# drwangxian/viterbi_spl

Hardware: AMD Instinct MI355X
Metric: Viterbi Mframes/s at S=361 T=30k; achieved HBM GB/s vs peak (higher is better)
Workload: dtype f32

## Files before the change

viterbi_spl_amd/csrc/banded.hip:

```cpp
#include "device_common.hpp"

namespace vit {

template <int W, int NWT, bool DW, bool DBG, int NXT, typename ET>
__global__ void __launch_bounds__((NWT + (DW ? 3 : 2)) * 64) banded_forward_kernel(FwdArgs a) {
    extern __shared__ __align__(16) unsigned char smem[];
    constexpr int NP = NWT * 64;
    constexpr int EPL = NWT;
    const int S = a.S, SP = a.SP, T = a.T, SD = a.SD;
    constexpr int DC = NP + 16;
    float* dls = reinterpret_cast<float*>(smem);
    float* dl = dls + 4;
    float* Pv = dls + 4 * DC;
    float* Sv = Pv + NP + 1;
    float* Dv = Sv + NP + 1;
    VI* tot = reinterpret_cast<VI*>(Dv + kMaxDenseRows);

    const int tid = threadIdx.x;
    const int lane = tid & 63;
    const int wv = __builtin_amdgcn_readfirstlane(tid >> 6);
    const int song = blockIdx.x;
    const int Tb = song_length(a.lengths, song, T);
    const ET* __restrict__ E = reinterpret_cast<const ET*>(a.logE) + (size_t)song * T * S;
    float* __restrict__ hist = a.hist + (size_t)song * T * SD;
// ... 182 lines not shown
        }
        const unsigned long long s3 = prof ? stamp() : 0ull;
        __syncthreads();
        if (prof) {
            const unsigned long long s4 = stamp();
            ph0 += s1 - s0; ph1 += s2 - s1; ph2 += s3 - s2; ph3 += s4 - s3;
        }
    };
    const unsigned long long clk0 = (dbg & 48) ? __builtin_amdgcn_s_memtime() : 0ull;
    const unsigned long long rt0 = (dbg & 48) ? __builtin_amdgcn_s_memrealtime() : 0ull;
    int t = 1;
    for (; t + 1 < Tb; t += 2) {
        frame(t, e_a);
        frame(t + 1, e_b);
    }
    if (t < Tb) frame(t, e_a);

    terminal_argmax(is_target ? dl[j] : -INFINITY, j, tvalid, tot, NWT + (DW ? 3 : 2), a.last_state, a.loglik, song);
    if ((dbg & 256) && lane == 0 && Tb > 1) {
        float* o = a.fmax + (size_t)song * 64 + 4 * wv;
        const float n = (float)(Tb - 1);
        o[0] = (float)ph0 / n; o[1] = (float)ph1 / n; o[2] = (float)ph2 / n; o[3] = (float)ph3 / n;
    }
    if ((dbg & 48) && tid == 0) {
        const unsigned long long d = (dbg & 16) ? __builtin_amdgcn_s_memtime() - clk0 : __builtin_amdgcn_s_memrealtime() - rt0;
        a.fmax[(size_t)song * 64 + 63] = (float)d / (float)(Tb > 1 ? Tb - 1 : 1);
    }
}

#include "banded_floor.inc"

constexpr int split_waitcnt(int vm, int lgkm) { return (vm & 15) | ((vm >> 4) << 14) | (7 << 4) | (lgkm << 8); }
constexpr int kNoVmWait = 63;
template <int... K, typename F>
__device__ __forceinline__ void split_frames(std::integer_sequence<int, K...>, F&& f) { (f(std::integral_constant<int, K>{}), ...); }
template <int NXT, int PF, typename ET, bool WPR = false, bool XQ = false>
__global__ void __launch_bounds__(64 * (kSplitFullWaves + kSplitHalfWaves)) banded_floor_split_forward_kernel(FwdArgs a) {
    extern __shared__ __align__(16) unsigned char smem[];
    constexpr int W = 32;
    constexpr int NWF = kSplitFullWaves, NW = kSplitFullWaves + kSplitHalfWaves;
    using L = FloorSplitLds;
    constexpr int DC = L::DC, BUF = L::BUF;
    float* dls = reinterpret_cast<float*>(smem) + L::dls;
    float* fmg = dls + L::fmg;
    VI* tot = reinterpret_cast<VI*>(dls + L::tot);
    const int S = a.S, SP = a.SP, T = a.T, SD = a.SD;
    constexpr bool GEN = NXT < 0;
    constexpr int NXL = GEN ? kMaxExtras : NXT;
    const int nx = GEN ? a.n_extras : NXT;

    const int tid = threadIdx.x;
    const int lane = tid & 63;
    const int wv = __builtin_amdgcn_readfirstlane(tid >> 6);
    const bool half = wv >= NWF;
    const int hh = half ? lane >> 5 : 0;
    const int song = blockIdx.x;
    const int Tb = song_length(a.lengths, song, T);
    const ET* __restrict__ E = reinterpret_cast<const ET*>(a.logE) + (size_t)song * T * S;
    float* __restrict__ hist = a.hist + (size_t)song * T * SD;

    const int j = half ? 64 * NWF + 32 * (wv - NWF) + (lane & 31) : tid;
    const bool tvalid = j < S;
    const bool own = tvalid && hh == 0;
    const int jc = tvalid ? j : 0;
    const int jld = tvalid ? j : S - 1;
    const bool is_fm = j == S;
    const unsigned hoff = tvalid ? (unsigned)(SD + j) : (is_fm ? (unsigned)S : (unsigned)(SD + S + 1));
    const unsigned hoffb = 4u * hoff, eoffb = (unsigned)(sizeof(ET) * jld);
    const int lo = reinterpret_cast<const int32_t*>(a.image + a.off_lo)[jc];
    int xcol[NXL > 0 ? NXL : 1];
    bool is_x = false;
#pragma unroll
    for (int k = 0; k < NXL; ++k) {
        xcol[k] = k < nx ? a.extras[k] : 0;
        is_x |= (k < nx && j == xcol[k]);
    }
    const int sh = a.win_shift;
    const int lov = (tvalid ? lo : 0) + sh;
    const float* rp = dls + 4 + (lov & 3) * DC + (lov & ~3) + 16 * hh;
    float* fmp = fmg + fm_slot((XQ && is_x) ? (lane | 1) : lane);
    static_assert(!XQ || NXT == 1, "the extra column leaves M by address only where the launcher proved its quad idle");

    for (int k = tid; k < L::reset; k += NW * 64) dls[k] = -INFINITY;
    __syncthreads();

#ifdef VIT_TIMING_HOOKS
    const bool probe = (a.debug & 48) != 0;
    constexpr bool wprobe = WPR;
    WaveProbe wp_;
#else
    constexpr bool probe = false;
#endif
    unsigned long long clk0 = 0ull, rt0 = 0ull;

    auto body = [&](auto role, auto resets) {
        constexpr bool HALF = decltype(role)::value, RESETS = decltype(resets)::value;
        constexpr int WL = HALF ? W / 2 : W;
        const float cj = own ? reinterpret_cast<const float*>(a.image + a.off_rowc)[jc] : -INFINITY;
        float aw[WL];
        float xa[NXL > 0 ? NXL : 1];
        {
            const float* __restrict__ tab = reinterpret_cast<const float*>(a.image + a.off_tabA);
            const float* __restrict__ xaT = reinterpret_cast<const float*>(a.image + a.off_extraA);
#pragma unroll
            for (int w = 0; w < WL; ++w) aw[w] = tvalid ? tab[(size_t)(w + (HALF ? 16 * hh : 0)) * SP + jc] : -INFINITY;
#pragma unroll
            for (int k = 0; k < NXL; ++k)
                xa[k] = (tvalid && k < nx && (!HALF || hh == 1)) ? xaT[(size_t)k * SP + jc] : -INFINITY;
        }
        float* wp = dls + 4 + sh + j + (HALF ? hh * split_upper_off(DC) : 0);
        int xo[NXL > 0 ? NXL : 1];
#pragma unroll
        for (int k = 0; k < NXL; ++k) {
            xo[k] = 4 + sh + xcol[k];
            asm volatile("" : "+v"(xo[k]));
        }

        auto produce = [&](const float dn, const int WB, const int G, const int Z) {
#pragma unroll
            for (int c = 0; c < (HALF ? 2 : 4); ++c) wp[WB * BUF + floor_copy_off(DC, c)] = dn;
            fm_publish(fmp + G * kFmGroupFloats, (!XQ && NXL > 0 && is_x) ? -INFINITY : dn);
            if constexpr (RESETS) fmg[Z * kFmGroupFloats + lane] = -INFINITY;
        };

        {
            const float d0 = tvalid ? reinterpret_cast<const float*>(a.image + a.off_logpi)[j] + load_e<ET>(E + j) : -INFINITY;
            if (own) hist[j] = d0;
            produce(d0, 0, 0, 1);
        }
        float er[PF];
#pragma unroll
        for (int k = 0; k < PF; ++k) er[k] = load_e<ET>(E + (size_t)(1 + k < Tb ? 1 + k : Tb - 1) * S + jld);
#pragma unroll
        for (int w = 0; w < WL; ++w) asm volatile("" ::"v"(aw[w]));
#pragma unroll
        for (int k = 0; k < NXL; ++k) asm volatile("" ::"v"(xa[k]));
        asm volatile("" ::"v"(cj));
        __syncthreads();

        const unsigned rowH = 4u * (unsigned)SD, rowE = (unsigned)sizeof(ET) * (unsigned)S;
        float* hb = hist;
        const ET* eb = E;
        unsigned elim = 0;
        auto round_bases = [&](const int t) {
            const int r = t + PF < Tb ? t + PF : Tb - 1;
            const int ahead = Tb - 1 - r < PF ? Tb - 1 - r : PF;
            hb = hist + (size_t)(t - 1) * SD;
            eb = E + (size_t)r * S;
            elim = (unsigned)ahead * rowE;
        };
        auto frame = [&](float& e_slot, auto uc) {
            constexpr int u = decltype(uc)::value;
            const int RB = u & 1, WB = RB ^ 1;
            const int GR = u % kFmGroups, GW = (u + 1) % kFmGroups, GZ = (u + 2) % kFmGroups;
            const f32x4* __restrict__ win = reinterpret_cast<const f32x4*>(rp + RB * BUF);
            float xd[NXL > 0 ? NXL : 1];
            f32x4 fq;
            float m0, m1 = -INFINITY, m2 = -INFINITY, m3 = -INFINITY;
#pragma unroll
            for (int k = 0; k < NXL; ++k) xd[k] = dls[xo[k] + RB * BUF];
            fq = reinterpret_cast<const f32x4*>(fmg + GR * kFmGroupFloats)[0];
            asm volatile("" ::: "memory");
            f32x4 dw[WL / 4];
#pragma unroll
            for (int q = 0; q < WL / 4; ++q) dw[q] = win[q];
            __builtin_amdgcn_sched_barrier(0);
            const float M = fmaxf(fmaxf(fq.x, fq.y), fmaxf(fq.z, fq.w));
            m0 = M + cj;
            asm volatile("" ::"v"(m0));
            __builtin_amdgcn_sched_barrier(0);
            split_frames(std::make_integer_sequence<int, WL / 8>{}, [&](auto gc) {
                constexpr int w = 8 * decltype(gc)::value;
                constexpr bool last = w + 8 == WL;
                constexpr int vmw = PF - 1 + u;
                static_assert(vmw <= 2 * (PF - 1) && 2 * (PF - 1) < kNoVmWait, "vmcnt bound: one store and one load per frame, 6-bit field");
                constexpr bool pairw = w + 16 >= WL && w >= 8;
                f32x4 da = dw[w / 4], db = dw[w / 4 + 1];
                if constexpr (pairw) {
                    __builtin_amdgcn_s_waitcnt(split_waitcnt(last ? vmw : kNoVmWait, last ? 0 : 2));
                    asm volatile("" : "+v"(da), "+v"(db));
                }
                f32x2 c0_ = f32x2{da.x, da.y} + f32x2{aw[w + 0], aw[w + 1]};
                f32x2 c1_ = f32x2{da.z, da.w} + f32x2{aw[w + 2], aw[w + 3]};
                f32x2 c2_ = f32x2{db.x, db.y} + f32x2{aw[w + 4], aw[w + 5]};
                f32x2 c3_ = f32x2{db.z, db.w} + f32x2{aw[w + 6], aw[w + 7]};
                asm volatile("" : "+v"(c0_), "+v"(c1_), "+v"(c2_), "+v"(c3_));
                m0 = fmaxf(fmaxf(m0, c0_.x), c0_.y);
                m1 = fmaxf(fmaxf(m1, c1_.x), c1_.y);
                m2 = fmaxf(fmaxf(m2, c2_.x), c2_.y);
                m3 = fmaxf(fmaxf(m3, c3_.x), c3_.y);
            });
#pragma unroll
            for (int k = 0; k < NXL; ++k) m1 = fmaxf(m1, xd[k] + xa[k]);
            float mx = fmaxf(fmaxf(m0, m1), fmaxf(m2, m3));
            if constexpr (HALF) mx = max_other_half(mx);
            const float dn = mx + e_slot;
#ifdef VIT_TIMING_HOOKS
            if constexpr (wprobe) wp_.before_publish(dn);
#endif
            const float sv = (HALF && is_fm) ? M : dn;
            const unsigned eso = (unsigned)u * rowE < elim ? (unsigned)u * rowE : elim;
            produce(dn, WB, GW, GZ);
            asm volatile("" ::: "memory");
            row_store_f32(hb, hoffb, sv, (unsigned)u * rowH);
            e_slot = row_load_e<ET>(eb, eoffb, eso);
#ifdef VIT_TIMING_HOOKS
            if constexpr (wprobe) wp_.barrier(); else
#endif
            __syncthreads();
        };
#ifdef VIT_TIMING_HOOKS
        if constexpr (wprobe) wp_.start();
#endif
        clk0 = probe ? __builtin_amdgcn_s_memtime() : 0ull;
        rt0 = probe ? __builtin_amdgcn_s_memrealtime() : 0ull;
        if constexpr (HALF) __builtin_amdgcn_s_setprio(1);
        int t = 1;
        for (; t + PF - 1 < Tb; t += PF) {
            round_bases(t);
            split_frames(std::make_integer_sequence<int, PF>{}, [&](auto k) { frame(er[k], k); });
        }
        round_bases(t);
        split_frames(std::make_integer_sequence<int, PF - 1>{}, [&](auto k) {
            if (t + k < Tb) frame(er[k], k);
        });
    };
    static_assert(PF % 2 == 0 && PF % kFmGroups == 0, "the unrolled frames must cycle through whole buffer and slot-group rounds");
// ... 194 lines not shown
        __syncthreads();
        if (tid == 0) {
            VI acc = vi_identity();
            for (int b = 0; b < NPW; ++b) acc = op_fwd(acc, tot[b]);
            if (acc.i == kBig) acc.i = 0;
            a.last_state[song] = acc.i;
            if (a.loglik) a.loglik[song] = acc.v;
        }
    }
    if (probe && tid == 0) {
        const unsigned long long d = (a.debug & 16) ? __builtin_amdgcn_s_memtime() - clk0 : __builtin_amdgcn_s_memrealtime() - rt0;
        a.fmax[(size_t)song * 64 + 63] = (float)d / (float)(Tb > 1 ? Tb - 1 : 1);
    }
}

__global__ void scan_selftest_kernel(const float* __restrict__ vals, int mode, float* __restrict__ out_v,
                                     int32_t* __restrict__ out_i) {
    const int j = threadIdx.x + blockIdx.x * blockDim.x;
    VI x{vals[j], (int)threadIdx.x};
    if (mode == 0) x = wave_scan<false>(x);
    else if (mode == 1) x = wave_scan<true>(x);
    else if (mode == 2) x.v = wave_scan_max(x.v);
    else if (mode == 3) x.v = wave_shift_up(wave_scan_max(x.v), -INFINITY);
    else x.v = wave_max_all(x.v);
    out_v[j] = x.v;
    out_i[j] = x.i;
}

template <int W, int NWT, typename ET>
static hipError_t launch_floor_t(const FwdArgs& a, hipStream_t st) {
    constexpr int PF = floor_pf<W>();
    if constexpr (W == 32 && NWT == 6) {
        static_assert(kSplitStates == NWT * 64, "the split kernel keeps the six-wave kernel's LDS and history layout");
        if (a.fwd_form == 6 || (a.fwd_form == 0 && a.B <= 256 && std::is_same_v<ET, float>)) {
            constexpr size_t ldss = FloorSplitLds::bytes();
            constexpr int NWS = kSplitFullWaves + kSplitHalfWaves;
            const bool xq = a.n_extras == 1 && a.extras[0] == a.S - 1 && (a.S - 1) % 4 == 0;
#ifdef VIT_TIMING_HOOKS
            if ((a.debug & 64) && xq)
                hipLaunchKernelGGL((banded_floor_split_forward_kernel<1, PF, ET, true, true>), dim3((int)a.B), dim3(NWS * 64), ldss, st, a);
            else if ((a.debug & 64) && a.n_extras == 1)
                hipLaunchKernelGGL((banded_floor_split_forward_kernel<1, PF, ET, true>), dim3((int)a.B), dim3(NWS * 64), ldss, st, a);
            else
#endif
            if (xq)
                hipLaunchKernelGGL((banded_floor_split_forward_kernel<1, PF, ET, false, true>), dim3((int)a.B), dim3(NWS * 64), ldss, st, a);
            else if (a.n_extras == 1)
                hipLaunchKernelGGL((banded_floor_split_forward_kernel<1, PF, ET>), dim3((int)a.B), dim3(NWS * 64), ldss, st, a);
            else
                hipLaunchKernelGGL((banded_floor_split_forward_kernel<-1, PF, ET>), dim3((int)a.B), dim3(NWS * 64), ldss, st, a);
            return hipGetLastError();
        }
    }
    if constexpr (W <= 32 && NWT <= 8) {
        const bool pair = a.pair_ok && ((a.B > 256 && a.fwd_form != 1 && a.fwd_form != 6) || a.fwd_form == 2);
        if (pair) {
            constexpr int NPW = (NWT + 1) / 2;
            constexpr int PFP = 4;
            constexpr size_t ldsp = FloorPairLds<NPW>::bytes();
            if (W == 32 && a.n_extras == 1)
                hipLaunchKernelGGL((banded_floor_pair_forward_kernel<W, NPW, (W == 32 ? 1 : -1), PFP, ET>), dim3((int)a.B), dim3(NPW * 64), ldsp, st, a);
            else
                hipLaunchKernelGGL((banded_floor_pair_forward_kernel<W, NPW, -1, PFP, ET>), dim3((int)a.B), dim3(NPW * 64), ldsp, st, a);
            return hipGetLastError();
        }
    }
    constexpr size_t ldsf = FloorLds<W, NWT>::bytes();
#ifdef VIT_TIMING_HOOKS
    if constexpr (W == 32 && NWT == 6) {
        if ((a.debug & 64) && a.n_extras == 1) {
            hipLaunchKernelGGL((banded_floor_forward_kernel<W, NWT, 1, PF, ET, WgVariant::Plain, true>), dim3((int)a.B), dim3(NWT * 64), ldsf, st, a);
            return hipGetLastError();
        }
    }
#endif
    return with_nxt<W>(a.n_extras, [&](auto nxt) {
        hipLaunchKernelGGL((banded_floor_forward_kernel<W, NWT, decltype(nxt)::value, PF, ET>), dim3((int)a.B), dim3(NWT * 64), ldsf, st, a);
        return hipGetLastError();
    });
}

// ... 63 lines not shown
```

viterbi_spl_amd/csrc/capi.hip:

```cpp
#include <hip/hip_runtime.h>

#include <algorithm>
#include <cstdlib>
#include <cstring>
#include <functional>
#include <mutex>
#include <queue>
#include <new>
#include <utility>
#include <vector>

#include "../../include/viterbi_hip.h"
#include "kernels.hpp"
#include "plan.hpp"

struct Tuning {
    int forward_form = 0;
    int backtrace_form = 0;
    int dense_songs = 0;
    int dense_one_thread = 0;
    int dense_form = 0;
    int step_form = 0;
    int bt_chunks = 0;
    int bt_warm = -1;
    int win_shift = -1;
    int wave_min_batch = 0;
    int wave_two = 0;
    int wave_uniform = 0;
    int bt_fast_rows = 0;
    int bt_block_waves = 0;
    int wave_history = 0;
    int timing = 0;
};

enum Family : int {
    kFamNone = 0,
    kFamStep = 1,
    kFamGroup = 2,
    kFamWave = 3,
};
inline hipError_t launch_family(int family, vit::WgVariant v, const vit::FwdArgs& a, bool f16, hipStream_t st) {
    if (family == kFamWave) return vit::launch_wave(a, f16, st);
    return family == kFamGroup ? vit::launch_banded_variant(a, v, f16, st) : vit::launch_step_variant(a, v, f16, st);
}

struct HistLayout {
    int SD = 0;
    int col0 = 0, mcol = 0;
    int xcol0 = -1;
    int have_fmax = 0;
};

struct FwdStamp {
    const void* ws = nullptr;
    int64_t B = 0, T = 0;
    int family = 0;
    HistLayout lay;
    int aux_frames = 1;
    int half = 0;
    const void* logE = nullptr;
    int e_f16 = 0;
};

// ... 209 lines not shown
    info->reserved[2] = (plan->bp.ok && plan->bp.lo_affine ? 1 : 0) | (plan->bp.ok && plan->bp.pair_ok ? 2 : 0) |
                        (plan->bp.step_ok && vit::step_kernel_instantiated(plan->S, plan->bp.step_bw, plan->bp.step_kb) ? 4 : 0) |
                        (plan->bp.ok && plan->bp.wave_ok ? 8 : 0);
    info->consts[0] = plan->bp.c0;
    for (int k = 0; k < vit::kMaxExtras; ++k) info->extras[k] = k < plan->bp.n_extras ? plan->bp.extras[k] : -1;
    return VIT_OK;
}

size_t vit_plan_image_bytes(const vit_plan* plan) { return plan ? plan->L.bytes : 0; }

int vit_plan_upload(vit_plan* plan, void* device_image, size_t bytes, vit_stream stream) {
    if (!plan || !device_image) return VIT_EINVAL;
    if (bytes < plan->L.bytes || ((uintptr_t)device_image & 255) != 0) return VIT_EINVAL;
    VIT_TRY(hipMemcpyAsync(device_image, plan->host_image.data(), plan->L.bytes, hipMemcpyHostToDevice, (hipStream_t)stream));
    plan->dev_image = static_cast<const uint8_t*>(device_image);
    int dev = 0, cus = 0;
    if (hipGetDevice(&dev) == hipSuccess && hipDeviceGetAttribute(&cus, hipDeviceAttributeMultiprocessorCount, dev) == hipSuccess && cus > 0)
        plan->n_cus = cus;
    return VIT_OK;
}

size_t vit_workspace_bytes(const vit_plan* plan, int64_t B, int64_t T) {
    if (!plan || B < 0 || T < 1) return 0;
    return ws_layout(plan, B, T).bytes;
}

static int* tuning_field(Tuning& t, const char* key) {
    struct { const char* k; int Tuning::*f; } const tab[] = {
        {"forward_form", &Tuning::forward_form}, {"backtrace_form", &Tuning::backtrace_form},
        {"dense_songs", &Tuning::dense_songs}, {"dense_one_thread", &Tuning::dense_one_thread}, {"dense_form", &Tuning::dense_form},
        {"step_form", &Tuning::step_form}, {"bt_chunks", &Tuning::bt_chunks}, {"bt_warm", &Tuning::bt_warm},
        {"win_shift", &Tuning::win_shift}, {"wave_min_batch", &Tuning::wave_min_batch}, {"wave_two", &Tuning::wave_two},
        {"bt_fast_rows", &Tuning::bt_fast_rows}, {"bt_block_waves", &Tuning::bt_block_waves}, {"wave_history", &Tuning::wave_history}, {"wave_uniform", &Tuning::wave_uniform},
        {"timing", &Tuning::timing},
    };
    for (const auto& e : tab)
        if (std::strcmp(e.k, key) == 0) return &(t.*(e.f));
    return nullptr;
}

int vit_plan_set_option(vit_plan* plan, const char* key, int64_t value) {
    if (!plan || !key) return VIT_EINVAL;
    if (std::strcmp(key, "reset") == 0) { plan->tune = Tuning(); return VIT_OK; }
    int* f = tuning_field(plan->tune, key);
    if (!f || value < -1 || value > (int64_t)1 << 30) return VIT_EINVAL;
#ifndef VIT_TIMING_HOOKS
    if (f == &plan->tune.timing && value != 0) return VIT_EUNSUPPORTED;
#endif
    *f = (int)value;
    return VIT_OK;
}

static int resolve_family(const vit_plan* plan, int algo, int64_t B) {
    const int nwt = vit::banded_waves_for(plan->S);
    const bool group_ok = plan->bp.ok && (vit::scan_form_instantiated(plan->bp.W, nwt) ||
                                          (plan->bp.floor_ok && plan->S < nwt * 64 && vit::floor_form_instantiated(plan->bp.W, nwt)));
    const bool wave_ok = plan->bp.ok && plan->bp.wave_ok;
    const int ff = plan->tune.forward_form;
    const int64_t wmin = plan->tune.wave_min_batch > 0 ? plan->tune.wave_min_batch : wave_min_batch(plan);
    if (algo == VIT_ALGO_DENSE) return kFamStep;
    if (algo == VIT_ALGO_WAVE) return wave_ok ? kFamWave : VIT_EUNSUPPORTED;
    if (algo == VIT_ALGO_GROUP) return group_ok ? kFamGroup : VIT_EUNSUPPORTED;
    if (algo != VIT_ALGO_AUTO && algo != VIT_ALGO_BANDED) return VIT_EINVAL;
    const bool want_wave = wave_ok && ff != 5 && (ff == 4 || (ff == 0 && B >= wmin) || !group_ok);
    if (want_wave) return kFamWave;
    if (group_ok) return kFamGroup;
    return algo == VIT_ALGO_AUTO ? kFamStep : VIT_EUNSUPPORTED;
// ... 13 lines not shown
    a.c0 = plan->bp.c0;
    a.debug = tn.timing;
    a.fwd_form = (tn.forward_form >= 1 && tn.forward_form <= 3) || tn.forward_form == 6 ? tn.forward_form : 0;
    a.dense_kt1 = tn.dense_one_thread;
    a.dense_form = tn.dense_form;
    a.step_form = tn.step_form;
    a.off_logpi = plan->L.off_logpi;
    a.off_A4 = plan->L.off_A4;
    a.off_lo = plan->L.off_lo;
    a.off_kind = plan->L.off_kind;
    a.off_tabA = plan->L.off_tabA;
    a.off_extraA = plan->L.off_extraA;
    a.off_denseA = plan->L.off_denseA;
    a.off_rowc = plan->L.off_rowc;
    a.off_lo2 = plan->L.off_lo2;
    a.off_tabP = plan->L.off_tabP;
    a.pair_ok = plan->bp.ok && plan->bp.pair_ok ? 1 : 0;
    a.floor_ok = plan->bp.ok && plan->bp.floor_ok ? 1 : 0;
    a.step_ok = plan->bp.step_ok ? 1 : 0;
    a.step_bw = plan->bp.step_bw;
    a.step_kb = plan->bp.step_kb;
    a.step_cn = plan->bp.step_cn;
    a.off_stepC = plan->L.off_stepC;
    a.off_Arow = plan->L.off_Arow;
    a.off_tabV = plan->L.off_tabV;
    a.wave_ok = plan->bp.ok && plan->bp.wave_ok ? 1 : 0;
    a.wave_npl = plan->bp.wave_npl;
    a.wave_dk = plan->bp.wave_dk;
    a.wave_u5 = tn.wave_uniform == 1 ? 0 : (tn.wave_uniform == 2 ? (plan->wave_u5 >= 1 ? 1 : 0) : (tn.wave_uniform == 3 && plan->wave_u5 == 2 ? 3 : plan->wave_u5));
    a.wave_flags = ((tn.wave_two & 3) == 1 ? 1 : ((tn.wave_two & 3) == 2 ? 2 : 0)) | (tn.wave_two & 4);
    a.win_shift = (plan->bp.ok && plan->bp.lo_affine) ? (plan->bp.lo_off & 3) : 0;
    a.win_shift2 = (plan->bp.ok && plan->bp.pair_ok && plan->bp.lo2_affine) ? (plan->bp.lo2_off & 3) : 0;
    if (tn.win_shift >= 0) a.win_shift = a.win_shift2 = tn.win_shift & 3;
}

size_t vit_workspace_bytes_for(const vit_plan* plan, int64_t B, int64_t T, int algo) {
    if (!plan || B < 0 || T < 1) return 0;
    const int family = resolve_family(plan, algo, B);
    if (family < 0) return 0;
    return ws_layout_family(plan, family, B, T).bytes;
}

int vit_forward(const vit_plan* plan, const void* logE, int emis_dtype, int64_t B, int64_t T,
                const int64_t* lengths, void* workspace, size_t workspace_bytes, float* loglik, int algo,
                vit_stream stream) {
    int rc = check_common(plan, B, T, workspace);
    if (rc != VIT_OK) return rc;
    if (!logE) return VIT_EINVAL;
    if (emis_dtype != VIT_F32 && emis_dtype != VIT_F16) return VIT_EINVAL;
    const int family = resolve_family(plan, algo, B);
    if (family < 0) return family;
    const Tuning& tn = plan->tune;
    const bool half = family == kFamWave && wave_half_applies(plan, T);
    if (family == kFamWave && tn.wave_history == 2 && !half && T >= 2) return VIT_EUNSUPPORTED;
    const WsLayout w = ws_layout_family(plan, family, B, T);
    if (workspace_bytes < w.bytes) return VIT_EWORKSPACE;
    if (B == 0) return VIT_OK;
    stamp_erase(plan, workspace);

    uint8_t* ws = static_cast<uint8_t*>(workspace);
    vit::FwdArgs a{};
    fwd_args_from_plan(plan, a);
    a.logE = logE;
    a.lengths = lengths;
    a.hist = reinterpret_cast<float*>(ws + w.off_hist);
    a.fmax = reinterpret_cast<float*>(ws + w.off_fmax);
// ... 900 lines not shown
```

viterbi_spl_amd/csrc/kernels.hpp:

```cpp
#pragma once
#include <hip/hip_runtime.h>

#include <cstdint>

#include "plan.hpp"

namespace vit {

constexpr int banded_waves_for(int S) {
    const int need = (S + 63) / 64;
    const int opts[5] = {2, 4, 6, 8, 12};
    for (int k = 0; k < 5; ++k)
        if (opts[k] >= need) return opts[k];
    return 0;
}
constexpr bool scan_form_instantiated(int W, int nwt) { return nwt > 0 && ((W <= 32 && nwt <= 12) || (W == 64 && nwt <= 6)); }
constexpr bool floor_form_instantiated(int W, int nwt) { return nwt > 0 && W <= 128 && nwt <= 12; }
constexpr int banded_target_waves(int S, int W) {
    const int nwt = banded_waves_for(S);
    return scan_form_instantiated(W, nwt) ? nwt : 0;
}
enum class WgVariant { Plain, Packed, Ckpt, PackedCkpt };
constexpr bool floor_packed_applies(int S, int W, bool floor_ok, int n_dense) {
    const int nwt = banded_waves_for(S);
// ... 19 lines not shown
    int T, S, SP, S4, SD, W;
    int n_extras, n_dense;
    int extras[kMaxExtras];
    float c0;
    int debug;
    int fwd_form;
    int dense_kt1;
    int dense_form;
    int step_form;
    size_t off_logpi, off_A4, off_lo, off_kind, off_tabA, off_extraA, off_denseA, off_rowc, off_lo2, off_tabP;
    int pair_ok;
    int floor_ok;
    int step_ok, step_bw, step_kb;
    float step_cn;
    size_t off_stepC, off_Arow;
    int win_shift2;
    size_t off_tabV;
    int wave_ok, wave_npl, wave_dk;
    int wave_u5;
    int wave_flags;
    int hist_half;
    int64_t hist_rows;
    int ckpt_every, t_begin, t_end;
    const float* init_rows;
    int64_t init_stride;
    const int64_t* offsets;
    int n_slots;
    const int32_t* slot_begin;
    const int32_t* slot_songs;
    const int64_t* ckpt_base;
    const int32_t* unit_song;
    const int32_t* unit_seg;
    int win_shift;
};

struct BtArgs {
    const uint8_t* image;
    const float* hist;
    const int32_t* last_state;
    const int64_t* lengths;
    int32_t* states;
    int32_t* entry;
    int64_t B;
    int T, S, SP, SD, W, K;
    int col0, mcol;
    int xcol0;
    int aux_frames;
    int chunks, warm;
    int banded;
    int have_fmax;
    int bt_form;
    int lo_affine, lo_off;
    int dense_rows[kMaxDenseRows];
    int n_extras, n_dense;
    int extras[kMaxExtras];
    float c0;
    size_t off_lo, off_kind, off_tabA, off_extraA, off_denseA, off_Arow, off_rowc, off_tabX, off_stepC;
    int step_ok, step_kb, step_mult;
    float step_cn;
    int hist_half;
    int64_t hist_rows;
    int mcol_odd, xcol0_odd;
    const void* logE;
    int e_f16;
    int64_t states_stride;
    int block_waves;
// ... 90 lines not shown
```

viterbi_spl_amd/csrc/plan.cpp:

```cpp
#include "plan.hpp"

#include <algorithm>
#include <cmath>
#include <cstring>
#include <limits>
#include <map>
#include <queue>
#include <utility>

namespace vit {

static inline uint32_t f2u(float f) {
    uint32_t u;
    std::memcpy(&u, &f, 4);
    return u;
}

static inline size_t align256(size_t x) { return (x + 255) & ~size_t(255); }

BandedPlan analyze_banded(const float* A, int S) {
    BandedPlan bp;
    bp.S = S;
    bp.SP = (S + 63) / 64 * 64;
    bp.lo.assign(bp.SP, 0);
// ... 82 lines not shown
    }
    for (int off = 0; off <= W && !bp.lo_affine; ++off) {
        bool all = true;
        for (int j = 0; j < S && all; ++j)
            if (bp.kind[j] == -1) all = bp.lo[j] == std::max(0, std::min(j - off, S - W));
        if (all) { bp.lo_affine = true; bp.lo_off = off; }
    }
    {
        bp.lo2.assign(bp.SP / 2, 0);
        bool ok = bp.n_dense == 0;
        for (int p = 0; p < (S + 1) / 2 && ok; ++p) {
            const int j0 = 2 * p, j1 = std::min(2 * p + 1, S - 1);
            const int l = std::min(lo[j0], lo[j1]), h = std::max(hi[j0], hi[j1]);
            if (h - l + 1 > W) { ok = false; break; }
            bp.lo2[p] = std::max(0, std::min(l, S - W));
        }
        bp.pair_ok = ok;
        for (int off = 0; off <= 2 * W && ok && !bp.lo2_affine; ++off) {
            bool all = true;
            for (int p = 0; p < (S + 1) / 2 && all; ++p) all = bp.lo2[p] == std::max(0, std::min(2 * p - off, S - W));
            if (all) { bp.lo2_affine = true; bp.lo2_off = off; }
        }
    }
    {
        bool ok = bp.n_dense == 0;
        for (int j = 0; j < S && ok; ++j) {
            const float cj = bp.rowc[j];
            for (int w = 0; w < W && ok; ++w) {
                const int i = bp.lo[j] + w;
                if (!is_extra(i) && !(A[(size_t)j * S + i] >= cj)) ok = false;
            }
        }
        bp.floor_ok = ok;
    }
    {
        bool ok = bp.floor_ok;
        for (int j = 0; j < S && ok; ++j)
            for (int k = 0; k < bp.n_extras && ok; ++k)
                if (!(A[(size_t)j * S + bp.extras[k]] >= bp.rowc[j])) ok = false;
        bp.floor_all_ok = ok;
        int d = 0;
        for (int j = 0; j < S; ++j) d = std::max(d, std::max(j - lo[j], hi[j] - j));
        bp.wave_d = d;
        bp.wave_npl = (S + 63) / 64;
        bp.wave_dk = wave_table_d(bp.wave_npl, d);
        bp.wave_ok = ok && bp.n_dense == 0 && bp.n_extras <= kWaveMaxExtras && bp.wave_dk > 0 && S + bp.n_extras < 64 * bp.wave_npl;
    }
    bp.ok = true;
    return bp;
}

void analyze_step(const float* A, int S, BandedPlan& bp) {
    bp.step_ok = false;
    const int n = S - 1, SP = bp.SP;
    if (n < 128) return;
    int bw = 1;
    while (bw < n && f2u(A[(size_t)bw * S]) == f2u(A[0])) ++bw;
    if (bw < 4 || bw > 64) return;
    int kb = 0;
    for (int j = 0; j < n;) {
        int r = j;
        while (r < n && f2u(A[(size_t)r * S]) == f2u(A[(size_t)j * S])) ++r;
        if (r == n) break;
        if (r - j != bw) return;
        ++kb;
        j = r;
    }
    if (kb < 1 || kb > kMaxStepBands || (kb + 1) * bw >= n) return;
    std::vector<float> C((size_t)(kMaxStepBands + 1) * SP, -std::numeric_limits<float>::infinity());
    std::vector<char> have((size_t)(kb + 1) * n, 0);
    for (int i = 0; i < n; ++i)
        for (int j = 0; j < n; ++j) {
            const int d = i > j ? i - j : j - i;
            const int k = std::min(d / bw, kb);
            const float v = A[(size_t)j * S + i];
            if (f2u(v) != f2u(v) || (f2u(v) & 0x7fffffffu) > 0x7f800000u) return;
            if (!have[(size_t)k * n + i]) { have[(size_t)k * n + i] = 1; C[(size_t)k * SP + i] = v; }
            else if (f2u(C[(size_t)k * SP + i]) != f2u(v)) return;
        }
    for (int i = 0; i < n; ++i)
        for (int k = 0; k <= kb; ++k) {
            if (!have[(size_t)k * n + i]) C[(size_t)k * SP + i] = C[(size_t)kb * SP + i];
// ... 157 lines not shown
```

viterbi_spl_amd/csrc/plan.hpp:

```cpp
#pragma once
#include <cstddef>
#include <cstdint>
#include <vector>

namespace vit {

constexpr int kMaxExtras = 4;
constexpr int kMaxDenseRows = 4;
inline constexpr int kBandedWidths[] = {16, 32, 64, 84, 96, 128};
constexpr bool banded_width_instantiated(int W) {
    for (int w : kBandedWidths)
        if (w == W) return true;
    return false;
}

struct BandedPlan {
    bool ok = false;
    int S = 0;
    int SP = 0;
    float c0 = 0.f;
    std::vector<float> rowc;
    int n_extras = 0;
    int extras[kMaxExtras] = {0, 0, 0, 0};
    int n_dense = 0;
    int dense_rows[kMaxDenseRows] = {0, 0, 0, 0};
    int max_window = 0;
    int W = 0;
    std::vector<int32_t> lo;
    std::vector<int32_t> kind;
    bool lo_affine = false;
    bool floor_ok = false;
    bool pair_ok = false;
    std::vector<int32_t> lo2;
    bool lo2_affine = false;
    int lo2_off = 0;
    int lo_off = 0;

    bool step_ok = false;
    int step_bw = 0, step_kb = 0;
    std::vector<float> stepC;
    float step_cn = 0.f;

    bool floor_all_ok = false;
    bool wave_ok = false;
    int wave_npl = 0;
    int wave_d = 0;
    int wave_dk = 0;
};

constexpr int kWaveMaxExtras = 2;
constexpr int wave_table_d(int npl, int d) { return (npl == 6 && d <= 14) ? 14 : 0; }
constexpr int wave_pairs(int dk) { return dk + 1; }
constexpr int wave_halo(int npl, int dk) { return (dk + npl - 1) / npl; }
constexpr int wave_p0e(int npl, int dk, int k) { return (k + npl * wave_halo(npl, dk) - dk) & ~1; }

constexpr int kMaxStepBands = 15;
void analyze_step(const float* logA_T, int S, BandedPlan& bp);

BandedPlan analyze_banded(const float* logA_T, int S);

struct ImageLayout {
    int S = 0, SP = 0, S4 = 0, W = 0, n_extras = 0, n_dense = 0;
    size_t off_logpi = 0;
    size_t off_A4 = 0;
    size_t off_lo = 0;
    size_t off_kind = 0;
    size_t off_tabA = 0;
    size_t off_extraA = 0;
    size_t off_denseA = 0;
    size_t off_Arow = 0;
    size_t off_rowc = 0;
    size_t off_lo2 = 0;
    size_t off_tabP = 0;
    size_t off_tabX = 0;
    size_t off_stepC = 0;
    size_t off_tabV = 0;
    size_t bytes = 0;
};

struct PackedCkptSchedule {
    std::vector<int32_t> unit_song, unit_seg;
    std::vector<int64_t> launch_begin, ckpt_base;
};
int64_t packed_ckpt_units(const int64_t* offsets, int64_t B, int64_t K);
void packed_ckpt_schedule(const int64_t* offsets, int64_t B, int64_t K, int64_t max_units, PackedCkptSchedule& out);

ImageLayout make_layout(int S, const BandedPlan& bp);
void fill_image(const float* logA_T, const float* log_pi, const BandedPlan& bp,
                const ImageLayout& L, uint8_t* image);

}
```

viterbi_spl_amd/csrc/plan_host_capi.cpp:

```cpp
#include <cstring>
#include <vector>

#include "plan.hpp"

extern "C" {

struct vph_plan {
    vit::BandedPlan bp;
    vit::ImageLayout L;
    std::vector<uint8_t> image;
};

vph_plan* vph_create(const float* logA_T, const float* log_pi, int S) {
    vph_plan* p = new vph_plan();
    p->bp = vit::analyze_banded(logA_T, S);
    if (!p->bp.ok) vit::analyze_step(logA_T, S, p->bp);
    p->L = vit::make_layout(S, p->bp);
    p->image.resize(p->L.bytes);
    vit::fill_image(logA_T, log_pi, p->bp, p->L, p->image.data());
    return p;
}
void vph_destroy(vph_plan* p) { delete p; }

void vph_info(const vph_plan* p, int* info, float* c0) {
    info[0] = p->bp.ok; info[1] = p->bp.S; info[2] = p->bp.SP; info[3] = p->bp.W;
    info[4] = p->bp.n_extras; info[5] = p->bp.n_dense; info[6] = p->bp.max_window;
    for (int k = 0; k < 4; ++k) { info[7 + k] = p->bp.extras[k]; info[11 + k] = p->bp.dense_rows[k]; }
    info[15] = p->L.S4 | (p->bp.pair_ok ? 0x10000 : 0) | (p->bp.floor_ok ? 0x20000 : 0) | (p->bp.step_ok ? 0x40000 : 0) |
               ((p->bp.step_ok ? p->bp.step_kb : 0) << 20) | ((p->bp.step_ok ? p->bp.step_bw : 0) << 24);
    *c0 = p->bp.c0;
}
void vph_offsets(const vph_plan* p, long long* off) {
    off[0] = p->L.off_logpi; off[1] = p->L.off_A4; off[2] = p->L.off_lo; off[3] = p->L.off_kind;
    off[4] = p->L.off_tabA; off[5] = p->L.off_extraA; off[6] = p->L.off_denseA; off[7] = p->L.bytes;
    off[8] = p->L.off_Arow; off[9] = p->L.off_rowc; off[10] = p->L.off_lo2; off[11] = p->L.off_tabP;
}
void vph_wave(const vph_plan* p, long long* w) {
    w[0] = p->bp.wave_ok; w[1] = p->bp.wave_npl; w[2] = p->bp.wave_d; w[3] = p->bp.wave_dk;
    w[4] = p->bp.floor_all_ok; w[5] = (long long)p->L.off_tabV;
}
void vph_step(const vph_plan* p, long long* s, float* cn) {
    s[0] = p->bp.step_ok; s[1] = p->bp.step_ok ? p->bp.step_bw : 0; s[2] = p->bp.step_ok ? p->bp.step_kb : 0;
    s[3] = (long long)p->L.off_stepC;
    *cn = p->bp.step_ok ? p->bp.step_cn : 0.f;
}
void vph_image(const vph_plan* p, unsigned char* out) { std::memcpy(out, p->image.data(), p->image.size()); }

long long vph_packed_ckpt_schedule(const long long* offsets, long long B, long long K, long long max_units, int* unit_song, int* unit_seg,
                                   long long cap_units, long long* launch_begin, long long cap_launches, long long* ckpt_base) {
    std::vector<int64_t> off(offsets, offsets + B + 1);
    const int64_t units = vit::packed_ckpt_units(off.data(), B, K);
    if (units < 0 || units > cap_units) return -1;
    vit::PackedCkptSchedule sc;
    vit::packed_ckpt_schedule(off.data(), B, K, max_units, sc);
    const long long nl = (long long)sc.launch_begin.size() - 1;
    if (nl > cap_launches) return -1;
    for (size_t u = 0; u < sc.unit_song.size(); ++u) { unit_song[u] = sc.unit_song[u]; unit_seg[u] = sc.unit_seg[u]; }
    for (size_t l = 0; l < sc.launch_begin.size(); ++l) launch_begin[l] = sc.launch_begin[l];
    for (size_t b = 0; b < sc.ckpt_base.size(); ++b) ckpt_base[b] = sc.ckpt_base[b];
    return nl;
}

}
```

Baseline: 490.5.

## Trim split-kernel full-wave window to the live transition width

Measured after the change: 497.0 (median of 6 runs). 1.3% higher.

```diff
diff --git a/viterbi_spl_amd/csrc/banded.hip b/viterbi_spl_amd/csrc/banded.hip
--- a/viterbi_spl_amd/csrc/banded.hip
+++ b/viterbi_spl_amd/csrc/banded.hip
@@ -238,12 +238,14 @@
 
 constexpr int split_waitcnt(int vm, int lgkm) { return (vm & 15) | ((vm >> 4) << 14) | (7 << 4) | (lgkm << 8); }
 constexpr int kNoVmWait = 63;
+constexpr int split_reads_behind(int NQ, int g) { return (NQ + 1) - 2 * (g + 1); }
 template <int... K, typename F>
 __device__ __forceinline__ void split_frames(std::integer_sequence<int, K...>, F&& f) { (f(std::integral_constant<int, K>{}), ...); }
-template <int NXT, int PF, typename ET, bool WPR = false, bool XQ = false>
+template <int NXT, int PF, typename ET, bool WPR = false, bool XQ = false, int WF = 32>
 __global__ void __launch_bounds__(64 * (kSplitFullWaves + kSplitHalfWaves)) banded_floor_split_forward_kernel(FwdArgs a) {
     extern __shared__ __align__(16) unsigned char smem[];
     constexpr int W = 32;
+    static_assert(WF == W || (WF % 4 == 1 && WF >= 9 && WF < W && NXT == 1), "a trimmed window: whole quads and one float, one extra column");
     constexpr int NWF = kSplitFullWaves, NW = kSplitFullWaves + kSplitHalfWaves;
     using L = FloorSplitLds;
     constexpr int DC = L::DC, BUF = L::BUF;
@@ -301,7 +303,8 @@
 
     auto body = [&](auto role, auto resets) {
         constexpr bool HALF = decltype(role)::value, RESETS = decltype(resets)::value;
-        constexpr int WL = HALF ? W / 2 : W;
+        constexpr int WL = HALF ? W / 2 : WF;
+        constexpr bool TRIM = WL % 4 != 0;
         const float cj = own ? reinterpret_cast<const float*>(a.image + a.off_rowc)[jc] : -INFINITY;
         float aw[WL];
         float xa[NXL > 0 ? NXL : 1];
@@ -362,7 +365,7 @@
             const f32x4* __restrict__ win = reinterpret_cast<const f32x4*>(rp + RB * BUF);
             float xd[NXL > 0 ? NXL : 1];
             f32x4 fq;
-            float m0, m1 = -INFINITY, m2 = -INFINITY, m3 = -INFINITY;
+            [[maybe_unused]] float m0, m1 = -INFINITY, m2 = -INFINITY, m3 = -INFINITY;
 #pragma unroll
             for (int k = 0; k < NXL; ++k) xd[k] = dls[xo[k] + RB * BUF];
             fq = reinterpret_cast<const f32x4*>(fmg + GR * kFmGroupFloats)[0];
@@ -370,35 +373,95 @@
             f32x4 dw[WL / 4];
 #pragma unroll
             for (int q = 0; q < WL / 4; ++q) dw[q] = win[q];
+            [[maybe_unused]] float ds = 0.f;
+            if constexpr (TRIM) ds = (rp + RB * BUF)[WL - 1];
             __builtin_amdgcn_sched_barrier(0);
+            if constexpr (TRIM) {
+                static_assert(split_reads_behind(WL / 4, 0) == WL / 4 + 1 - 2, "behind the first pair: every other window read of the burst");
+                __builtin_amdgcn_s_waitcnt(split_waitcnt(kNoVmWait, split_reads_behind(WL / 4, 0)));
+                asm volatile("" : "+v"(fq), "+v"(dw[0]), "+v"(dw[1]));
+            }
             const float M = fmaxf(fmaxf(fq.x, fq.y), fmaxf(fq.z, fq.w));
             m0 = M + cj;
             asm volatile("" ::"v"(m0));
             __builtin_amdgcn_sched_barrier(0);
-            split_frames(std::make_integer_sequence<int, WL / 8>{}, [&](auto gc) {
-                constexpr int w = 8 * decltype(gc)::value;
-                constexpr bool last = w + 8 == WL;
-                constexpr int vmw = PF - 1 + u;
-                static_assert(vmw <= 2 * (PF - 1) && 2 * (PF - 1) < kNoVmWait, "vmcnt bound: one store and one load per frame, 6-bit field");
-                constexpr bool pairw = w + 16 >= WL && w >= 8;
-                f32x4 da = dw[w / 4], db = dw[w / 4 + 1];
-                if constexpr (pairw) {
-                    __builtin_amdgcn_s_waitcnt(split_waitcnt(last ? vmw : kNoVmWait, last ? 0 : 2));
-                    asm volatile("" : "+v"(da), "+v"(db));
+            float mx;
+            constexpr int vmw = PF - 1 + u;
+            static_assert(vmw <= 2 * (PF - 1) && 2 * (PF - 1) < kNoVmWait, "vmcnt bound: one store and one load per frame, 6-bit field");
+            if constexpr (TRIM) {
+                constexpr int NQ = WL / 4, TQ = NQ % 2 ? 1 : 2, NPB = (NQ - TQ) / 2;
+                static_assert(NXL == 1 && NQ >= 3 && 2 * NPB + TQ == NQ && 4 * NQ + 1 == WL, "pairs of quads, then the tail: one or two quads and one float");
+                static_assert(split_reads_behind(NQ, 0) <= 15, "lgkmcnt is a four-bit field");
+                static_assert(split_reads_behind(NQ, NPB - 1) == TQ + 1, "behind the last pair stand the tail's reads -- TQ quads and the float -- and nothing else");
+                static_assert(split_reads_behind(NQ, NPB) + 2 == TQ + 1 && TQ <= 2, "the tail's wait, lgkmcnt(0), leaves no window read out");
+                float mb = xd[0] + xa[0];
+                asm volatile("" ::"v"(mb));
+                split_frames(std::make_integer_sequence<int, NPB>{}, [&](auto gc) {
+                    constexpr int w = 8 * decltype(gc)::value;
+                    f32x4 da = dw[w / 4], db = dw[w / 4 + 1];
+                    if constexpr (decltype(gc)::value >= 1) {
+                        constexpr int behind = split_reads_behind(NQ, decltype(gc)::value);
+                        static_assert(behind >= TQ + 1 && behind + 2 == split_reads_behind(NQ, decltype(gc)::value - 1), "two reads fewer than the pair before");
+                        __builtin_amdgcn_s_waitcnt(split_waitcnt(kNoVmWait, behind));
+                        asm volatile("" : "+v"(da), "+v"(db));
+                    }
+                    f32x2 c0_ = f32x2{da.x, da.y} + f32x2{aw[w + 0], aw[w + 1]};
+                    f32x2 c1_ = f32x2{da.z, da.w} + f32x2{aw[w + 2], aw[w + 3]};
+                    f32x2 c2_ = f32x2{db.x, db.y} + f32x2{aw[w + 4], aw[w + 5]};
+                    f32x2 c3_ = f32x2{db.z, db.w} + f32x2{aw[w + 6], aw[w + 7]};
+                    asm volatile("" : "+v"(c0_), "+v"(c1_), "+v"(c2_), "+v"(c3_));
+                    m0 = fmaxf(fmaxf(m0, c0_.x), c0_.y);
+                    mb = fmaxf(fmaxf(mb, c1_.x), c1_.y);
+                    m0 = fmaxf(fmaxf(m0, c2_.x), c2_.y);
+                    mb = fmaxf(fmaxf(mb, c3_.x), c3_.y);
+                });
+                {
+                    constexpr int w = 8 * NPB;
+                    f32x4 da = dw[w / 4], db = dw[NQ - 1];
+                    __builtin_amdgcn_s_waitcnt(split_waitcnt(vmw, 0));
+                    if constexpr (TQ == 2) asm volatile("" : "+v"(da), "+v"(db), "+v"(ds)); else asm volatile("" : "+v"(da), "+v"(ds));
+                    f32x2 c0_ = f32x2{da.x, da.y} + f32x2{aw[w + 0], aw[w + 1]};
+                    f32x2 c1_ = f32x2{da.z, da.w} + f32x2{aw[w + 2], aw[w + 3]};
+                    float cs = ds + aw[WL - 1];
+                    if constexpr (TQ == 2) {
+                        f32x2 c2_ = f32x2{db.x, db.y} + f32x2{aw[w + 4], aw[w + 5]};
+                        f32x2 c3_ = f32x2{db.z, db.w} + f32x2{aw[w + 6], aw[w + 7]};
+                        asm volatile("" : "+v"(c0_), "+v"(c1_), "+v"(c2_), "+v"(c3_), "+v"(cs));
+                        m0 = fmaxf(fmaxf(m0, c0_.x), c0_.y);
+                        mb = fmaxf(fmaxf(mb, c1_.x), c1_.y);
+                        m0 = fmaxf(fmaxf(m0, c2_.x), c2_.y);
+                        mb = fmaxf(fmaxf(mb, c3_.x), c3_.y);
+                    } else {
+                        asm volatile("" : "+v"(c0_), "+v"(c1_), "+v"(cs));
+                        m0 = fmaxf(fmaxf(m0, c0_.x), c0_.y);
+                        mb = fmaxf(fmaxf(mb, c1_.x), c1_.y);
+                    }
+                    mx = fmaxf(fmaxf(m0, mb), cs);
                 }
-                f32x2 c0_ = f32x2{da.x, da.y} + f32x2{aw[w + 0], aw[w + 1]};
-                f32x2 c1_ = f32x2{da.z, da.w} + f32x2{aw[w + 2], aw[w + 3]};
-                f32x2 c2_ = f32x2{db.x, db.y} + f32x2{aw[w + 4], aw[w + 5]};
-                f32x2 c3_ = f32x2{db.z, db.w} + f32x2{aw[w + 6], aw[w + 7]};
-                asm volatile("" : "+v"(c0_), "+v"(c1_), "+v"(c2_), "+v"(c3_));
-                m0 = fmaxf(fmaxf(m0, c0_.x), c0_.y);
-                m1 = fmaxf(fmaxf(m1, c1_.x), c1_.y);
-                m2 = fmaxf(fmaxf(m2, c2_.x), c2_.y);
-                m3 = fmaxf(fmaxf(m3, c3_.x), c3_.y);
-            });
-#pragma unroll
-            for (int k = 0; k < NXL; ++k) m1 = fmaxf(m1, xd[k] + xa[k]);
-            float mx = fmaxf(fmaxf(m0, m1), fmaxf(m2, m3));
+            } else {
+                split_frames(std::make_integer_sequence<int, WL / 8>{}, [&](auto gc) {
+                    constexpr int w = 8 * decltype(gc)::value;
+                    constexpr bool last = w + 8 == WL;
+                    constexpr bool pairw = w + 16 >= WL && w >= 8;
+                    f32x4 da = dw[w / 4], db = dw[w / 4 + 1];
+                    if constexpr (pairw) {
+                        __builtin_amdgcn_s_waitcnt(split_waitcnt(last ? vmw : kNoVmWait, last ? 0 : 2));
+                        asm volatile("" : "+v"(da), "+v"(db));
+                    }
+                    f32x2 c0_ = f32x2{da.x, da.y} + f32x2{aw[w + 0], aw[w + 1]};
+                    f32x2 c1_ = f32x2{da.z, da.w} + f32x2{aw[w + 2], aw[w + 3]};
+                    f32x2 c2_ = f32x2{db.x, db.y} + f32x2{aw[w + 4], aw[w + 5]};
+                    f32x2 c3_ = f32x2{db.z, db.w} + f32x2{aw[w + 6], aw[w + 7]};
+                    asm volatile("" : "+v"(c0_), "+v"(c1_), "+v"(c2_), "+v"(c3_));
+                    m0 = fmaxf(fmaxf(m0, c0_.x), c0_.y);
+                    m1 = fmaxf(fmaxf(m1, c1_.x), c1_.y);
+                    m2 = fmaxf(fmaxf(m2, c2_.x), c2_.y);
+                    m3 = fmaxf(fmaxf(m3, c3_.x), c3_.y);
+                });
+#pragma unroll
+                for (int k = 0; k < NXL; ++k) m1 = fmaxf(m1, xd[k] + xa[k]);
+                mx = fmaxf(fmaxf(m0, m1), fmaxf(m2, m3));
+            }
             if constexpr (HALF) mx = max_other_half(mx);
             const float dn = mx + e_slot;
 #ifdef VIT_TIMING_HOOKS
@@ -659,21 +722,32 @@
     constexpr int PF = floor_pf<W>();
     if constexpr (W == 32 && NWT == 6) {
         static_assert(kSplitStates == NWT * 64, "the split kernel keeps the six-wave kernel's LDS and history layout");
+        static_assert(kSplitFullRows == 64 * kSplitFullWaves, "FwdArgs::floor_live speaks for the full waves' targets");
         if (a.fwd_form == 6 || (a.fwd_form == 0 && a.B <= 256 && std::is_same_v<ET, float>)) {
             constexpr size_t ldss = FloorSplitLds::bytes();
             constexpr int NWS = kSplitFullWaves + kSplitHalfWaves;
             const bool xq = a.n_extras == 1 && a.extras[0] == a.S - 1 && (a.S - 1) % 4 == 0;
-#ifdef VIT_TIMING_HOOKS
-            if ((a.debug & 64) && xq)
-                hipLaunchKernelGGL((banded_floor_split_forward_kernel<1, PF, ET, true, true>), dim3((int)a.B), dim3(NWS * 64), ldss, st, a);
-            else if ((a.debug & 64) && a.n_extras == 1)
-                hipLaunchKernelGGL((banded_floor_split_forward_kernel<1, PF, ET, true>), dim3((int)a.B), dim3(NWS * 64), ldss, st, a);
-            else
-#endif
-            if (xq)
-                hipLaunchKernelGGL((banded_floor_split_forward_kernel<1, PF, ET, false, true>), dim3((int)a.B), dim3(NWS * 64), ldss, st, a);
-            else if (a.n_extras == 1)
-                hipLaunchKernelGGL((banded_floor_split_forward_kernel<1, PF, ET>), dim3((int)a.B), dim3(NWS * 64), ldss, st, a);
+            const int wf = split_full_width(a.floor_live, W, a.S, a.n_extras, !std::is_same_v<ET, float>);
+            auto go = [&](auto xqc, auto wfc) {
+                constexpr bool XQ = decltype(xqc)::value;
+                constexpr int WF = decltype(wfc)::value;
+#ifdef VIT_TIMING_HOOKS
+                if (a.debug & 64)
+                    hipLaunchKernelGGL((banded_floor_split_forward_kernel<1, PF, ET, true, XQ, WF>), dim3((int)a.B), dim3(NWS * 64), ldss, st, a);
+                else
+#endif
+                hipLaunchKernelGGL((banded_floor_split_forward_kernel<1, PF, ET, false, XQ, WF>), dim3((int)a.B), dim3(NWS * 64), ldss, st, a);
+            };
+            auto go_w = [&](auto xqc) {
+                if constexpr (std::is_same_v<ET, float>) {
+                    static_assert(sizeof(kSplitLiveWidths) / sizeof(int) == 2, "one case per instantiated live width");
+                    if (wf == 25) return go(xqc, std::integral_constant<int, 25>{});
+                    if (wf == 29) return go(xqc, std::integral_constant<int, 29>{});
+                }
+                return go(xqc, std::integral_constant<int, W>{});
+            };
+            if (xq) go_w(std::true_type{});
+            else if (a.n_extras == 1) go_w(std::false_type{});
             else
                 hipLaunchKernelGGL((banded_floor_split_forward_kernel<-1, PF, ET>), dim3((int)a.B), dim3(NWS * 64), ldss, st, a);
             return hipGetLastError();
diff --git a/viterbi_spl_amd/csrc/capi.hip b/viterbi_spl_amd/csrc/capi.hip
--- a/viterbi_spl_amd/csrc/capi.hip
+++ b/viterbi_spl_amd/csrc/capi.hip
@@ -29,6 +29,7 @@
     int wave_uniform = 0;
     int bt_fast_rows = 0;
     int bt_block_waves = 0;
+    int floor_live_window = 0;
     int wave_history = 0;
     int timing = 0;
 };
@@ -304,7 +305,7 @@
         {"step_form", &Tuning::step_form}, {"bt_chunks", &Tuning::bt_chunks}, {"bt_warm", &Tuning::bt_warm},
         {"win_shift", &Tuning::win_shift}, {"wave_min_batch", &Tuning::wave_min_batch}, {"wave_two", &Tuning::wave_two},
         {"bt_fast_rows", &Tuning::bt_fast_rows}, {"bt_block_waves", &Tuning::bt_block_waves}, {"wave_history", &Tuning::wave_history}, {"wave_uniform", &Tuning::wave_uniform},
-        {"timing", &Tuning::timing},
+        {"floor_live_window", &Tuning::floor_live_window}, {"timing", &Tuning::timing},
     };
     for (const auto& e : tab)
         if (std::strcmp(e.k, key) == 0) return &(t.*(e.f));
@@ -384,6 +385,7 @@
     a.win_shift = (plan->bp.ok && plan->bp.lo_affine) ? (plan->bp.lo_off & 3) : 0;
     a.win_shift2 = (plan->bp.ok && plan->bp.pair_ok && plan->bp.lo2_affine) ? (plan->bp.lo2_off & 3) : 0;
     if (tn.win_shift >= 0) a.win_shift = a.win_shift2 = tn.win_shift & 3;
+    a.floor_live = tn.floor_live_window == 0 ? vit::floor_live_width(plan->bp, vit::kSplitFullRows) : plan->bp.W;
 }
 
 size_t vit_workspace_bytes_for(const vit_plan* plan, int64_t B, int64_t T, int algo) {
diff --git a/viterbi_spl_amd/csrc/kernels.hpp b/viterbi_spl_amd/csrc/kernels.hpp
--- a/viterbi_spl_amd/csrc/kernels.hpp
+++ b/viterbi_spl_amd/csrc/kernels.hpp
@@ -75,6 +75,7 @@
     const int32_t* unit_song;
     const int32_t* unit_seg;
     int win_shift;
+    int floor_live;
 };
 
 struct BtArgs {
diff --git a/viterbi_spl_amd/csrc/plan.cpp b/viterbi_spl_amd/csrc/plan.cpp
--- a/viterbi_spl_amd/csrc/plan.cpp
+++ b/viterbi_spl_amd/csrc/plan.cpp
@@ -138,6 +138,12 @@
             }
         }
         bp.floor_ok = ok;
+        bp.live_last.assign(S, W - 1);
+        for (int j = 0; j < S && ok; ++j) {
+            int w = W - 1;
+            while (w >= 0 && (is_extra(bp.lo[j] + w) || f2u(A[(size_t)j * S + bp.lo[j] + w]) == row_mode[j])) --w;
+            bp.live_last[j] = w;
+        }
     }
     {
         bool ok = bp.floor_ok;
@@ -154,6 +160,13 @@
     }
     bp.ok = true;
     return bp;
+}
+
+int floor_live_width(const BandedPlan& bp, int n_rows) {
+    if (!bp.ok || !bp.floor_ok || bp.n_dense != 0 || (int)bp.live_last.size() < bp.S) return bp.W;
+    int last = 0;
+    for (int j = 0; j < n_rows && j < bp.S; ++j) last = std::max(last, (int)bp.live_last[j]);
+    return last + 1;
 }
 
 void analyze_step(const float* A, int S, BandedPlan& bp) {
diff --git a/viterbi_spl_amd/csrc/plan.hpp b/viterbi_spl_amd/csrc/plan.hpp
--- a/viterbi_spl_amd/csrc/plan.hpp
+++ b/viterbi_spl_amd/csrc/plan.hpp
@@ -30,6 +30,7 @@
     std::vector<int32_t> kind;
     bool lo_affine = false;
     bool floor_ok = false;
+    std::vector<int32_t> live_last;
     bool pair_ok = false;
     std::vector<int32_t> lo2;
     bool lo2_affine = false;
@@ -58,6 +59,15 @@
 void analyze_step(const float* logA_T, int S, BandedPlan& bp);
 
 BandedPlan analyze_banded(const float* logA_T, int S);
+int floor_live_width(const BandedPlan& bp, int n_rows);
+constexpr int kSplitFullRows = 256;
+inline constexpr int kSplitLiveWidths[] = {25, 29};
+constexpr int split_full_width(int live, int W, int S, int n_extras, bool f16) {
+    if (W != 32 || S <= kSplitFullRows || S >= 384 || n_extras != 1 || f16) return W;
+    for (int w : kSplitLiveWidths)
+        if (live >= 1 && live <= w && w < W) return w;
+    return W;
+}
 
 struct ImageLayout {
     int S = 0, SP = 0, S4 = 0, W = 0, n_extras = 0, n_dense = 0;
diff --git a/viterbi_spl_amd/csrc/plan_host_capi.cpp b/viterbi_spl_amd/csrc/plan_host_capi.cpp
--- a/viterbi_spl_amd/csrc/plan_host_capi.cpp
+++ b/viterbi_spl_amd/csrc/plan_host_capi.cpp
@@ -44,6 +44,10 @@
     s[3] = (long long)p->L.off_stepC;
     *cn = p->bp.step_ok ? p->bp.step_cn : 0.f;
 }
+int vph_live_width(const vph_plan* p, int n_rows) { return vit::floor_live_width(p->bp, n_rows); }
+int vph_split_full_width(const vph_plan* p, int f16) {
+    return vit::split_full_width(vit::floor_live_width(p->bp, vit::kSplitFullRows), p->bp.W, p->bp.S, p->bp.ok ? p->bp.n_extras : 0, f16 != 0);
+}
 void vph_image(const vph_plan* p, unsigned char* out) { std::memcpy(out, p->image.data(), p->image.size()); }
 
 long long vph_packed_ckpt_schedule(const long long* offsets, long long B, long long K, long long max_units, int* unit_song, int* unit_seg,
```
